# ljanyst/ssd-tensorflow

Hardware: AMD Instinct MI355X
Metric: images/sec (fwd+bwd) vgg300 batch32 (higher is better)
Workload: dtype f32; 1 GPU; vgg300 training step (forward + multibox loss + backward + momentum update), 32 images/GPU x 1 GPU, synthetic 300x300 BGR 0..255, GPU-encoded labels, Xavier-init weights (BASELINE.json configs[1]); global_batch=32, parallelism=dp1, allreduce=none

## Files before the change

### ssd_tensorflow_amd/csrc/api.hip

```cpp
#include "../../include/ssdvgg_hip.h"
#include "net.h"
#include "augment.h"
#include "annotate.h"
#include "jpeg.h"
#include "metrics.h"
#include <vector>
#include <map>
#include <memory>
#include <mutex>
#include <algorithm>

namespace ssd {
static thread_local std::string g_err;
void set_error(const char* fmt, ...) {
    char buf[1024];
    va_list ap;
    va_start(ap, fmt);
    vsnprintf(buf, sizeof buf, fmt, ap);
    va_end(ap);
    g_err = buf;
}
const char* get_error() { return g_err.c_str(); }

thread_local Profiler* g_prof = nullptr;
// ... 936 lines not shown
}
namespace {
struct WinoWs {
    float *U, *Uf, *V, *Mx, *Yt, *Ya, *slabs;
    size_t total;
    WinoWs(const ConvDesc& d, float* ws) {
        const size_t cop = wino_kpad(d.Co), u = (size_t)36 * d.Ci * cop, t = (size_t)36 * wino_tiles(d);
        U = ws; Uf = U + u; V = Uf + u; Mx = V + t * d.Ci; Yt = Mx + t * std::max((size_t)d.Ci, cop); Ya = Yt + t * cop; slabs = Ya + t * cop;
        total = (size_t)(slabs - ws) + wino_wgrad_ws_floats(d);
    }
};
}
size_t ssd_op_conv2d_wino_ws_floats(int b, int hi, int wi, int ci, int ho, int wo, int co, int kh, int kw, int stride, int dil,
                                    int pad_h, int pad_w) {
    const ConvDesc d = mk(b, hi, wi, ci, ho, wo, co, kh, kw, stride, dil, pad_h, pad_w);
    return wino_applicable(d) ? WinoWs(d, nullptr).total : 0;
}
size_t ssd_op_conv2d_wino_bits_words(int b, int hi, int wi, int ci, int ho, int wo, int co, int kh, int kw, int stride, int dil,
                                     int pad_h, int pad_w) {
    const ConvDesc d = mk(b, hi, wi, ci, ho, wo, co, kh, kw, stride, dil, pad_h, pad_w);
    return wino_applicable(d) ? (size_t)wino_tiles(d) * (d.Ci / 4) : 0;
}
int ssd_op_conv2d_wino_fwd(const float* x, const float* w, const float* bias, float* y, float* y_pool, void* rec, void* relu_bits, float* ws,
                           int flags, int b, int hi, int wi, int ci, int ho, int wo, int co, int kh, int kw, int stride, int dil,
                           int pad_h, int pad_w, int relu, void* stream) {
    API_BEGIN
    const ConvDesc d = mk(b, hi, wi, ci, ho, wo, co, kh, kw, stride, dil, pad_h, pad_w);
    SSD_REQUIRE(wino_applicable(d), "winograd: 3x3 / stride 1 / SAME layers (any dilation), Ci in multiples of 32, Co of 4");
    const WinoWs k(d, ws);
    if (!(flags & 1)) {
        HIP_OK(hipMemsetAsync(k.Uf, 0, (size_t)36 * d.Ci * wino_kpad(d.Co) * sizeof(float), (hipStream_t)stream));
        wino_filter(d, w, k.U, k.Uf, (hipStream_t)stream);
    }
    wino_fwd(d, x, k.U, bias, y, relu != 0, k.V, (size_t)wino_tiles(d) * d.Ci, k.Mx, y_pool, rec, (hipStream_t)stream, relu_bits);
    API_END
}
int ssd_op_conv2d_wino_dgrad(const float* dy, const float* w, float* dx, const float* mask, const void* mask_bits, int accumulate,
                             const void* rec, int uh, int uw, float* ws, int flags, int b, int hi, int wi, int ci, int ho, int wo, int co,
                             int kh, int kw, int stride, int dil, int pad_h, int pad_w, void* stream) {
    API_BEGIN
    const ConvDesc d = mk(b, hi, wi, ci, ho, wo, co, kh, kw, stride, dil, pad_h, pad_w);
    SSD_REQUIRE(wino_applicable(d), "winograd: 3x3 / stride 1 / SAME layers (any dilation), Ci in multiples of 32, Co of 4");
    const WinoWs k(d, ws);
    if (!(flags & 1)) {
        HIP_OK(hipMemsetAsync(k.Uf, 0, (size_t)36 * d.Ci * wino_kpad(d.Co) * sizeof(float), (hipStream_t)stream));
        wino_filter(d, w, k.U, k.Uf, (hipStream_t)stream);
    }
    wino_bwd_transform(d, dy, k.Yt, nullptr, (hipStream_t)stream);
    wino_dgrad(d, k.Yt, k.Uf, dx, mask, accumulate != 0, k.Mx, rec, uh, uw, (hipStream_t)stream, mask_bits);
    API_END
}
int ssd_op_conv2d_wino_wgrad(const float* x, const float* dy, float* dw, float* dbias, const float* w, float weight_decay, float* ws,
                             int flags, int b, int hi, int wi, int ci, int ho, int wo, int co, int kh, int kw, int stride, int dil,
                             int pad_h, int pad_w, void* stream) {
    API_BEGIN
    const ConvDesc d = mk(b, hi, wi, ci, ho, wo, co, kh, kw, stride, dil, pad_h, pad_w);
    SSD_REQUIRE(wino_applicable(d), "winograd: 3x3 / stride 1 / SAME layers (any dilation), Ci in multiples of 32, Co of 4");
    const WinoWs k(d, ws);
    const size_t vps = (size_t)wino_tiles(d) * d.Ci;
    if (!(flags & 2)) {
        ConvDesc dx = d;
        dx.Co = d.Ci; dx.Ho = d.Hi; dx.Wo = d.Wi;
        wino_bwd_transform(dx, x, k.V, nullptr, (hipStream_t)stream);
    }
    wino_bwd_transform(d, dy, nullptr, k.Ya, (hipStream_t)stream);
    wino_wgrad(d, k.V, vps, k.Ya, dw, dbias, w, weight_decay, k.slabs, (hipStream_t)stream);
    API_END
}
size_t ssd_op_conv2d_wgrad_ws_floats(int b, int hi, int wi, int ci, int ho, int wo, int co, int kh, int kw, int stride,
                                     int dil, int pad_h, int pad_w) {
    return conv_wgrad_ws_floats(mk(b, hi, wi, ci, ho, wo, co, kh, kw, stride, dil, pad_h, pad_w));
}
int ssd_op_conv2d_wgrad(const float* x, const float* dy, float* dw, float* dbias, const float* w, float weight_decay,
                        float* ws, int b, int hi, int wi, int ci, int ho, int wo, int co, int kh, int kw, int stride, int dil,
                        int pad_h, int pad_w, void* stream) {
    API_BEGIN
    conv_wgrad(mk(b, hi, wi, ci, ho, wo, co, kh, kw, stride, dil, pad_h, pad_w), x, dy, dw, dbias, w, weight_decay, ws,
               (hipStream_t)stream);
    API_END
}
int ssd_op_maxpool_fwd(const float* x, float* y, int b, int hi, int wi, int c, int ho, int wo, int k, int stride, int pad_h,
                       int pad_w, void* stream) {
// ... 167 lines not shown
```

### ssd_tensorflow_amd/csrc/conv.h

```cpp
#pragma once
#include <vector>
#include "common.h"

namespace ssd {

struct ConvDesc {
    int B, Hi, Wi, Ci;
    int Ho, Wo, Co;
    int KH, KW, stride, dil;
    int pad_h, pad_w;
};

void conv_fwd(const ConvDesc& d, const float* x, const float* w, const float* bias,
              float* y, bool relu, hipStream_t s);

void conv_dgrad(const ConvDesc& d, const float* dy, const float* w, float* dx,
                const float* mask, bool accumulate, hipStream_t s);

size_t conv_wgrad_ws_floats(const ConvDesc& d);
void conv_wgrad(const ConvDesc& d, const float* x, const float* dy, float* dw, float* dbias,
                const float* w, float weight_decay, float* ws, hipStream_t s);

bool conv_fwd_pool_supported(const ConvDesc& d);
void conv_fwd_pool(const ConvDesc& d, const float* x, const float* w, const float* bias, float* y_pool, void* rec, hipStream_t s);
bool conv_dgrad_unpool_supported(const ConvDesc& d);
void conv_dgrad_unpool(const ConvDesc& d, const float* dy, const float* w, float* dx_unpooled, const void* rec, int UH, int UW,
                       hipStream_t s);

bool conv_first_fwd_f32_applicable(const ConvDesc& d);
void conv_first_fwd_f32(const ConvDesc& d, const float* x, const float* w, const float* bias, float* y, bool relu, hipStream_t s);
bool conv_first_wgrad_f32_applicable(const ConvDesc& d);
size_t conv_first_wgrad_f32_ws_floats(const ConvDesc& d);
void conv_first_wgrad_f32(const ConvDesc& d, const float* x, const float* dy, float* dw, float* dbias, const float* w,
                          float weight_decay, float* ws, hipStream_t s);

bool wino_applicable(const ConvDesc& d);
int wino_tiles(const ConvDesc& d);
int wino_kpad(int c);
void wino_filter(const ConvDesc& d, const float* w, float* U, float* Uflip, hipStream_t s);
struct WinoFilterPlan {
    static constexpr int MAX = 24;
    struct Item {
        const float* w;
        float *U, *Uf;
        int Ci, Co, Cop, blk0;
    } it[MAX];
    int n = 0, blocks = 0;
    double elems = 0;
    void add(const float* w, float* U, float* Uf, int Ci, int Co);
};
void wino_filter_plan(const WinoFilterPlan& plan, bool forward, bool flipped, hipStream_t s);
size_t wino_fwd_ws_floats(const ConvDesc& d);
void wino_fwd(const ConvDesc& d, const float* x, const float* U, const float* bias, float* y, bool relu, float* V, size_t v_ps,
              float* Mws, float* y_pool, void* pool_rec, hipStream_t s, void* relu_bits = nullptr);
void wino_bwd_transform(const ConvDesc& d, const float* dy, float* Yt, float* Ya, hipStream_t s);
size_t wino_dgrad_ws_floats(const ConvDesc& d);
void wino_dgrad(const ConvDesc& d, const float* Yt, const float* Uflip, float* dx, const float* mask, bool accumulate, float* Xws,
                const void* unpool_rec, int UH, int UW, hipStream_t s, const void* mask_bits = nullptr);
size_t wino_wgrad_ws_floats(const ConvDesc& d);
void wino_wgrad(const ConvDesc& d, const float* V, size_t v_ps, const float* Ya, float* dw, float* dbias, const float* w,
                float weight_decay, float* ws, hipStream_t s);

bool conv_bigk(const ConvDesc& d);
double conv_bigk_useful_flops(const ConvDesc& d);
void conv_bigk_fwd(const ConvDesc& d, const float* x, const float* w, const float* bias, float* y, bool relu, hipStream_t s);
void conv_bigk_dgrad(const ConvDesc& d, const float* dy, const float* w, float* dx, const float* mask, bool accumulate, hipStream_t s);
void conv_bigk_wgrad(const ConvDesc& d, const float* x, const float* dy, float* dw, float* dbias, const float* w, float weight_decay,
                     hipStream_t s);

struct bf16_t;

void conv_fwd_smallc_bf16out(const ConvDesc& d, const float* x, const float* w, const float* bias, bf16_t* y, bool relu,
                             hipStream_t s);
void conv_wgrad_smallc_bf16dy(const ConvDesc& d, const float* x, const bf16_t* dy, float* dw, float* dbias, const float* w,
                              float weight_decay, float* ws, hipStream_t s);

void conv_first_fwd_bf16(const ConvDesc& d, const float* x, const float* w, const float* bias, bf16_t* y, bool relu, hipStream_t s);
size_t conv_first_wgrad_bf16_ws_floats(const ConvDesc& d);
void conv_first_wgrad_bf16(const ConvDesc& d, const float* x, const bf16_t* dy, float* dw, float* dbias, const float* w,
                           float weight_decay, float* ws, hipStream_t s);

void conv_bigk_fwd_bf16(const ConvDesc& d, const bf16_t* x, const bf16_t* w_oi, const float* bias, void* y, bool y_f32, bool relu,
                        hipStream_t s);
void conv_bigk_dgrad_bf16(const ConvDesc& d, const bf16_t* dy, const bf16_t* w_io, bf16_t* dx, const bf16_t* mask, bool accumulate,
                          hipStream_t s);
void conv_bigk_wgrad_bf16(const ConvDesc& d, const bf16_t* x, const bf16_t* dy, float* dw, float* dbias, const float* w,
                          float weight_decay, hipStream_t s);

struct FilterCastPlan {
    static constexpr int MAX_LAYERS = 48;
    struct Layer {
// ... 65 lines not shown
```

### ssd_tensorflow_amd/csrc/winograd.hip

```cpp
#include "conv.h"
#include "conv_detail.h"
#include "bf16.h"
#include <algorithm>
#include <cmath>

namespace ssd {

#define LDS_PTR(p) ((__attribute__((address_space(3))) void*)(p))
constexpr unsigned WOOB = 0xFFFFFFF0u;

__device__ __forceinline__ void bt6(f32x4& d0, f32x4& d1, f32x4& d2, f32x4& d3, f32x4& d4, f32x4& d5) {
    const f32x4 t0 = 1.265625f * d0 - 2.8125f * d2 + d4;
    const f32x4 e = d4 - 2.25f * d2, f = 1.6875f * d1 - 0.75f * d3;
    const f32x4 g = d4 - 0.5625f * d2, h = 0.84375f * d1 - 1.5f * d3;
    const f32x4 t5 = 1.265625f * d1 - 2.8125f * d3 + d5;
    d0 = t0; d1 = e - f; d2 = e + f; d3 = g - h; d4 = g + h; d5 = t5;
}
__device__ __forceinline__ void a6(const f32x4 e0, const f32x4 e1, const f32x4 e2, const f32x4 e3, f32x4* u) {
    const f32x4 p = e0 + 0.5625f * e2, q = 0.75f * e1 + 0.421875f * e3;
    const f32x4 r = e0 + 2.25f * e2, t = 1.5f * e1 + 3.375f * e3;
    u[0] = e0;
    u[1] = p + q;
    u[2] = p - q;
    u[3] = r + t;
    u[4] = r - t;
    u[5] = e3;
}
__device__ __forceinline__ void at4(const f32x4 m0, const f32x4 m1, const f32x4 m2, const f32x4 m3, const f32x4 m4, const f32x4 m5,
                                    f32x4* y) {
    const f32x4 s12 = m1 + m2, d12 = m1 - m2, s34 = m3 + m4, d34 = m3 - m4;
    y[0] = m0 + s12 + s34;
    y[1] = 0.75f * d12 + 1.5f * d34;
    y[2] = 0.5625f * s12 + 2.25f * s34;
    y[3] = 0.421875f * d12 + 3.375f * d34 + m5;
}

__host__ __device__ inline int bias_axis_slot(int k) { return k == 0 ? 0 : k == 1 ? 1 : k == 2 ? 2 : k == 5 ? 3 : -1; }
__device__ __forceinline__ float bias_axis_weight(int slot) {
    return slot == 0 ? -7.f / 9.f : slot == 1 ? 14.f / 9.f : slot == 2 ? 2.f / 9.f : 7.f / 16.f;
}

template <bool BT, bool AT>
__global__ __launch_bounds__(256) void wino_in_kernel(const float* __restrict__ x, float* __restrict__ V, float* __restrict__ Va,
                                                      int H, int W, int C, int Cp, int th, int tw, int T, unsigned x_bytes,
                                                      size_t v_ps, size_t va_ps, int D, unsigned long long* __restrict__ bits) {
    const int c4n = Cp >> 2;
    const int idx = blockIdx.x * 256 + threadIdx.x;
    const int q = idx % c4n, t = idx / c4n;
    if (t >= T) return;
    const int j = t % tw, t2 = t / tw;
    const int i = t2 % th, b = t2 / th;
    const int hb = (i % D) + D * 4 * (i / D), wb = (j % D) + D * 4 * (j / D);
    const __amdgpu_buffer_rsrc_t rs = __builtin_amdgcn_make_buffer_rsrc(const_cast<float*>(x), 0, x_bytes, 0x00020000);
    constexpr int LO = BT ? 0 : 1, HI = BT ? 6 : 5;
    f32x4 d[6][6];
#pragma unroll
    for (int r = LO; r < HI; ++r) {
        const int h = hb + D * (r - 1);
        const bool hv = (unsigned)h < (unsigned)H;
#pragma unroll
        for (int s = LO; s < HI; ++s) {
            const int w = wb + D * (s - 1);
            const bool ok = hv && (unsigned)w < (unsigned)W && q * 4 < C;
// ... 29 lines not shown
            a6(c[k][0], c[k][1], c[k][2], c[k][3], u);
#pragma unroll
            for (int l = 0; l < 6; ++l) *reinterpret_cast<f32x4*>(Va + (size_t)(k * 6 + l) * va_ps + row) = u[l];
        }
    }
    if constexpr (BT) {
#pragma unroll
        for (int s = 0; s < 6; ++s) bt6(d[0][s], d[1][s], d[2][s], d[3][s], d[4][s], d[5][s]);
#pragma unroll
        for (int r = 0; r < 6; ++r) {
            bt6(d[r][0], d[r][1], d[r][2], d[r][3], d[r][4], d[r][5]);
#pragma unroll
            for (int s = 0; s < 6; ++s) *reinterpret_cast<f32x4*>(V + (size_t)(r * 6 + s) * v_ps + row) = d[r][s];
        }
    }
}

struct WinoOutArgs {
    const float* M;
    size_t m_ps;
    float* y;
    const float* bias;
    const float* mask;
    const unsigned long long* mask_bits;
    int relu, accum;
    int H, W, N, th, tw, T;
    int D;
    unsigned short* pool_rec;
    int PH, PW;
    const unsigned short* unpool_rec;
    int UH, UW;
};

template <int MODE>
__global__ __launch_bounds__(256) void wino_out_kernel(WinoOutArgs p) {
    const int c4n = p.N >> 2;
    const int idx = blockIdx.x * 256 + threadIdx.x;
    const int q = idx % c4n, t = idx / c4n;
    if (t >= p.T) return;
    const int j = t % p.tw, t2 = t / p.tw;
    const int i = t2 % p.th, b = t2 / p.th;
    const int D = (MODE == 0 || MODE == 1) ? p.D : 1;
    const int hb = (i % D) + D * 4 * (i / D), wb = (j % D) + D * 4 * (j / D);
    const float* src = p.M + (size_t)t * p.N + q * 4;
    f32x4 c[4][6];
#pragma unroll
    for (int s = 0; s < 6; ++s) {
        f32x4 m[6];
#pragma unroll
        for (int r = 0; r < 6; ++r) m[r] = *reinterpret_cast<const f32x4*>(src + (size_t)(r * 6 + s) * p.m_ps);
        f32x4 y[4];
        at4(m[0], m[1], m[2], m[3], m[4], m[5], y);
#pragma unroll
        for (int r = 0; r < 4; ++r) c[r][s] = y[r];
    }
    f32x4 o[4][4];
#pragma unroll
    for (int r = 0; r < 4; ++r) at4(c[r][0], c[r][1], c[r][2], c[r][3], c[r][4], c[r][5], o[r]);

    if constexpr (MODE == 0 || MODE == 2) {
        const f32x4 bv = p.bias ? *reinterpret_cast<const f32x4*>(p.bias + q * 4) : f32x4{0.f, 0.f, 0.f, 0.f};
#pragma unroll
        for (int r = 0; r < 4; ++r)
#pragma unroll
            for (int s = 0; s < 4; ++s) {
                f32x4 v = o[r][s] + bv;
                if (p.relu) {
#pragma unroll
                    for (int e = 0; e < 4; ++e) v[e] = v[e] > 0.f ? v[e] : 0.f;
                }
                o[r][s] = v;
            }
    }
    if constexpr (MODE == 0) {
#pragma unroll
        for (int r = 0; r < 4; ++r) {
            const int h = hb + D * r;
            if (h >= p.H) continue;
#pragma unroll
            for (int s = 0; s < 4; ++s) {
                const int w = wb + D * s;
                if (w < p.W) *reinterpret_cast<f32x4*>(p.y + ((size_t)(b * p.H + h) * p.W + w) * p.N + q * 4) = o[r][s];
            }
        }
    } else if constexpr (MODE == 1) {
        const unsigned long long mbits = p.mask_bits ? p.mask_bits[(size_t)t * c4n + q] : 0ull;
#pragma unroll
        for (int r = 0; r < 4; ++r) {
            const int h = hb + D * r;
            if (h >= p.H) continue;
#pragma unroll
            for (int s = 0; s < 4; ++s) {
                const int w = wb + D * s;
                if (w >= p.W) continue;
                const size_t e0 = ((size_t)(b * p.H + h) * p.W + w) * p.N + q * 4;
                f32x4 v = o[r][s];
                if (p.accum) v += *reinterpret_cast<const f32x4*>(p.y + e0);
                if (p.mask_bits) {
                    const unsigned mb = (unsigned)(mbits >> ((r * 4 + s) * 4)) & 15u;
#pragma unroll
                    for (int e = 0; e < 4; ++e) v[e] = (mb >> e) & 1u ? v[e] : 0.f;
                } else if (p.mask) {
                    const f32x4 mk = *reinterpret_cast<const f32x4*>(p.mask + e0);
#pragma unroll
                    for (int e = 0; e < 4; ++e) v[e] = mk[e] > 0.f ? v[e] : 0.f;
                }
                *reinterpret_cast<f32x4*>(p.y + e0) = v;
            }
        }
    } else if constexpr (MODE == 2) {
#pragma unroll
        for (int wr = 0; wr < 2; ++wr) {
            const int ph = 2 * i + wr;
            if (ph >= p.PH) continue;
            const bool okh = 4 * i + 2 * wr + 1 < p.H;
#pragma unroll
            for (int wc = 0; wc < 2; ++wc) {
                const int pw = 2 * j + wc;
                if (pw >= p.PW) continue;
                const bool okw = 4 * j + 2 * wc + 1 < p.W;
                const bool ok[4] = {true, okw, okh, okw && okh};
                f32x4 mm = o[2 * wr][2 * wc];
                unsigned rec = 0;
#pragma unroll
                for (int e = 0; e < 4; ++e) {
                    unsigned a = 0;
                    float best = mm[e];
#pragma unroll
                    for (int cq = 1; cq < 4; ++cq) {
                        const float v = o[2 * wr + (cq >> 1)][2 * wc + (cq & 1)][e];
                        if (ok[cq] && v > best) { best = v; a = cq; }
                    }
                    mm[e] = best;
                    rec |= (a | (best > 0.f ? 4u : 0u)) << (3 * e);
                }
                const size_t pix = (size_t)(b * p.PH + ph) * p.PW + pw;
                *reinterpret_cast<f32x4*>(p.y + pix * p.N + q * 4) = mm;
                if (p.pool_rec) p.pool_rec[pix * c4n + q] = (unsigned short)rec;
            }
        }
    } else {
#pragma unroll
        for (int r = 0; r < 4; ++r) {
            const int h = 4 * i + r;
            if (h >= p.H) continue;
#pragma unroll
            for (int s = 0; s < 4; ++s) {
                const int w = 4 * j + s;
                if (w >= p.W) continue;
                const unsigned rec = p.unpool_rec[((size_t)(b * p.H + h) * p.W + w) * c4n + q];
#pragma unroll
                for (int cq = 0; cq < 4; ++cq) {
                    const int uh = 2 * h + (cq >> 1), uw = 2 * w + (cq & 1);
                    if (uh >= p.UH || uw >= p.UW) continue;
                    f32x4 v;
#pragma unroll
                    for (int e = 0; e < 4; ++e) {
                        const unsigned re = (rec >> (3 * e)) & 7u;
                        v[e] = ((re & 3u) == (unsigned)cq && (re & 4u)) ? o[r][s][e] : 0.f;
                    }
                    *reinterpret_cast<f32x4*>(p.y + ((size_t)(b * p.UH + uh) * p.UW + uw) * p.N + q * 4) = v;
                }
            }
        }
    }
}

__device__ __forceinline__ void g6(const float g0, const float g1, const float g2, float* u) {
    u[0] = (64.f / 81.f) * g0;
    const float a = (-128.f / 243.f) * g0 - (8.f / 27.f) * g2, b = (32.f / 81.f) * g1;
    u[1] = a - b;
    u[2] = a + b;
    const float c = (32.f / 243.f) * g0 + (8.f / 27.f) * g2, d = (16.f / 81.f) * g1;
    u[3] = c + d;
    u[4] = c - d;
    u[5] = g2;
}
template <bool FLIP>
__global__ __launch_bounds__(256) void wino_filter_kernel(WinoFilterPlan plan) {
    int li = 0;
    for (int k = 1; k < plan.n; ++k)
        if ((int)blockIdx.x >= plan.it[k].blk0) li = k;
    const float* __restrict__ w = plan.it[li].w;
    float* __restrict__ U = FLIP ? plan.it[li].Uf : plan.it[li].U;
    if (!U) return;
    const int Ci = plan.it[li].Ci, Co = plan.it[li].Co;
    const int idx = ((int)blockIdx.x - plan.it[li].blk0) * 256 + threadIdx.x;
    if (idx >= Ci * Co) return;
    const int ci = FLIP ? idx % Ci : idx / Co, co = FLIP ? idx / Ci : idx % Co;
    float g[3][3];
#pragma unroll
    for (int a = 0; a < 3; ++a)
#pragma unroll
        for (int b = 0; b < 3; ++b) g[a][b] = w[((size_t)((FLIP ? 2 - a : a) * 3 + (FLIP ? 2 - b : b)) * Ci + ci) * Co + co];
    float c[6][3];
#pragma unroll
    for (int b = 0; b < 3; ++b) {
        float u[6];
// ... 90 lines not shown
            for (int ni = 0; ni < TN; ++ni)
#pragma unroll
                for (int t = 0; t < 4; ++t) b[ni][t] = *reinterpret_cast<const float*>(S + b_col + ((kb + t) * BN + ni * 32) * 4);
#pragma unroll
            for (int t = 0; t < 4; ++t)
#pragma unroll
                for (int mi = 0; mi < TM; ++mi)
#pragma unroll
                    for (int ni = 0; ni < TN; ++ni)
                        acc[mi][ni] = __builtin_amdgcn_mfma_f32_32x32x2f32(a[mi][t], b[ni][t], acc[mi][ni], 0, 0, 0);
        }
    };
    if (nk > 0) issue(0, 0);
    for (int k = 0; k < nk; ++k) {
        asm volatile("s_waitcnt vmcnt(0)" ::: "memory");
        __builtin_amdgcn_s_barrier();
        asm volatile("" ::: "memory");
        if (k + 1 < nk) issue(k + 1, (k + 1) & 1);
        compute(k & 1);
    }
    float* const Cp = p.C + (size_t)pos * p.c_ps;
#pragma unroll
    for (int mi = 0; mi < TM; ++mi)
#pragma unroll
        for (int ni = 0; ni < TN; ++ni) {
            const int n = n0 + wn * 32 * TN + ni * 32 + li;
            if (n >= p.N) continue;
#pragma unroll
            for (int r = 0; r < 16; ++r) {
                const int m = m0 + wm * 32 * TM + mi * 32 + (r & 3) + 8 * (r >> 2) + 4 * lh;
                if (m < p.M) Cp[(size_t)m * p.N + n] = acc[mi][ni][r];
            }
        }
}

struct WinoTnArgs {
    const float* X;
    const float* Y;
    float* ws;
    int T, Ci, Co;
    int x_ld, y_ld;
    size_t x_ps, y_ps;
    int CT, NT, tchunk, nsplit;
};

template <int WM, int WN, int TM, int TN>
__global__ __launch_bounds__(256) void wino_gemm_tn_kernel(WinoTnArgs p) {
    constexpr int BKT = 32 * TM * WM, BNT = 32 * TN * WN, BP = 32;
    constexpr int XC = BKT / 4, YC = BNT / 4;
    constexpr int XRPP = 256 / XC, YRPP = 256 / YC;
    constexpr int X_N = BP / XRPP, Y_N = BP / YRPP;
    constexpr int X_BYTES = BP * BKT * 4, STAGE = BP * (BKT + BNT) * 4;
    static_assert(WM * WN == 4, "4 waves per workgroup");
    extern __shared__ __attribute__((aligned(16))) float smem[];
    unsigned char* const lds = reinterpret_cast<unsigned char*>(smem);
    const int tid = threadIdx.x;
    const int wave = __builtin_amdgcn_readfirstlane(tid >> 6), lane = tid & 63;
    int wg = xcd_remap(blockIdx.x, gridDim.x);
    const int nt = wg % p.NT;
    wg /= p.NT;
    const int ct = wg % p.CT;
    wg /= p.CT;
    const int split = wg % p.nsplit, pos = wg / p.nsplit;
    const int c0 = ct * BKT, n0 = nt * BNT;
    const int tbeg = split * p.tchunk, tend = min(p.T, tbeg + p.tchunk);
    const int niter = (tend - tbeg + BP - 1) / BP;
// ... 220 lines not shown
    static bool once = (set_lds(kern, lds), true);
    (void)once;
    a.MT = cdiv(a.M, BM);
    a.NT = cdiv(a.N, BN);
    ProfScope prof(label, 2.0 * 36 * a.M * (double)a.N * a.K, 4.0 * 36 * ((double)a.M * a.K + (double)a.K * a.N + (double)a.M * a.N), s);
    hipLaunchKernelGGL(kern, dim3(36 * a.MT * a.NT), dim3(256), lds, s, a);
    HIP_OK(hipGetLastError());
}

static void gemm_nn(const float* A, size_t a_ps, const float* Bm, float* C, size_t c_ps, int M, int N, int K, hipStream_t s) {
    WinoGemmArgs a{};
    a.A = A; a.Bm = Bm; a.C = C; a.M = M; a.N = N; a.K = K;
    a.a_ps = a_ps; a.b_ps = (size_t)K * N; a.c_ps = c_ps;
    static const int forced = env_int("SSD_WINO_TILE", -1);
    int cfg = 0;
    if (forced >= 0) cfg = forced;
    else if (cdiv(N, 64) * 64 < cdiv(N, 128) * 128) cfg = 1;
    else if ((double)cdiv(M, 128) * 128 > 1.06 * M && (double)cdiv(M, 64) * 64 < (double)cdiv(M, 128) * 128) cfg = 2;
    switch (cfg) {
    case 0: launch_nn<2, 2, 2, 2>(a, "wino_gemm_128x128", s); break;
    case 1: launch_nn<4, 1, 1, 2>(a, "wino_gemm_128x64", s); break;
    case 2: launch_nn<2, 2, 1, 2>(a, "wino_gemm_64x128", s); break;
    default: launch_nn<2, 2, 1, 1>(a, "wino_gemm_64x64", s); break;
    }
}

template <int MODE>
static void launch_out(WinoOutArgs& a, const char* label, double bytes, hipStream_t s) {
    ProfScope prof(label, 0, bytes, s);
    SSD_LAUNCH_STOP(wino_out_kernel<MODE>, dim3(cdiv((long long)a.T * (a.N / 4), 256)), dim3(256), 0, s, a);
    HIP_OK(hipGetLastError());
}

size_t wino_fwd_ws_floats(const ConvDesc& d) { return (size_t)36 * wino_tiles(d) * d.Co; }

void wino_fwd(const ConvDesc& d, const float* x, const float* U, const float* bias, float* y, bool relu, float* V, size_t v_ps,
              float* Mws, float* y_pool, void* pool_rec, hipStream_t s, void* relu_bits) {
    require(d);
    const int T = wino_tiles(d);
    launch_in(x, V, nullptr, d.B, d.Hi, d.Wi, d.Ci, d.Ci, d.dil, v_ps, 0, s, static_cast<unsigned long long*>(relu_bits));
    gemm_nn(V, v_ps, U, Mws, (size_t)T * d.Co, T, d.Co, d.Ci, s);
    WinoOutArgs a{};
    a.M = Mws; a.m_ps = (size_t)T * d.Co; a.bias = bias; a.relu = relu; a.H = d.Ho; a.W = d.Wo; a.N = d.Co;
    a.th = tiles_1d(d.Ho, d.dil); a.tw = tiles_1d(d.Wo, d.dil); a.T = T; a.D = d.dil;
    const double mb = 4.0 * 36 * T * d.Co;
    if (y_pool) {
        SSD_REQUIRE(d.dil == 1, "winograd: the fused pool is for undilated layers");
        a.y = y_pool; a.pool_rec = static_cast<unsigned short*>(pool_rec); a.PH = (d.Ho + 1) / 2; a.PW = (d.Wo + 1) / 2;
        launch_out<2>(a, "wino_out_pool", mb + 4.0 * d.B * a.PH * a.PW * d.Co, s);
    } else {
        a.y = y;
        launch_out<0>(a, "wino_out", mb + 4.0 * d.B * d.Ho * d.Wo * d.Co, s);
    }
}

size_t wino_dgrad_ws_floats(const ConvDesc& d) { return (size_t)36 * wino_tiles(d) * d.Ci; }

void wino_bwd_transform(const ConvDesc& d, const float* dy, float* Yt, float* Ya, hipStream_t s) {
    require(d);
    const size_t ps = (size_t)wino_tiles(d) * wino_kpad(d.Co);
    launch_in(dy, Yt, Ya, d.B, d.Ho, d.Wo, d.Co, wino_kpad(d.Co), d.dil, ps, ps, s);
}

void wino_dgrad(const ConvDesc& d, const float* Yt, const float* Uflip, float* dx, const float* mask, bool accumulate, float* Xws,
                const void* unpool_rec, int UH, int UW, hipStream_t s, const void* mask_bits) {
    require(d);
    const int T = wino_tiles(d);
    gemm_nn(Yt, (size_t)T * wino_kpad(d.Co), Uflip, Xws, (size_t)T * d.Ci, T, d.Ci, wino_kpad(d.Co), s);
    WinoOutArgs a{};
    a.M = Xws; a.m_ps = (size_t)T * d.Ci; a.y = dx; a.mask = mask; a.accum = accumulate; a.H = d.Hi; a.W = d.Wi; a.N = d.Ci;
    a.mask_bits = mask ? static_cast<const unsigned long long*>(mask_bits) : nullptr;
    a.th = tiles_1d(d.Hi, d.dil); a.tw = tiles_1d(d.Wi, d.dil); a.T = T; a.D = d.dil;
    const double mb = 4.0 * 36 * T * d.Ci;
    if (unpool_rec) {
        SSD_REQUIRE(d.dil == 1, "winograd: the un-pooling form is for undilated layers");
        a.unpool_rec = static_cast<const unsigned short*>(unpool_rec); a.UH = UH; a.UW = UW;
        launch_out<3>(a, "wino_out_unpool", mb + 4.0 * d.B * UH * UW * d.Ci, s);
    } else {
        launch_out<1>(a, "wino_out_dgrad", mb + 4.0 * d.B * d.Hi * d.Wi * d.Ci * (mask && !a.mask_bits ? 2 : 1), s);
    }
}

static void tn_tile(const ConvDesc& d, int* bk, int* bn) {
    *bk = d.Ci <= 64 ? 64 : 128;
    *bn = d.Co <= 64 ? 64 : 128;
}
static int tn_splits(const ConvDesc& d) {
    const int T = wino_tiles(d);
    int bk, bn;
    tn_tile(d, &bk, &bn);
    const int base = 36 * cdiv(d.Ci, bk) * cdiv(d.Co, bn);
    const double slots = 256.0 * std::min(8, (int)(160 * 1024 / (2 * 32 * (bk + bn) * 4)));
    const double it_us = 3.4 * (bk * bn) / (128.0 * 128.0) * slots / 512.0;
    int best = 1;
    double bc = 1e300;
    for (int ns = 1; ns <= 16; ++ns) {
        const int chunk = cdiv(cdiv(T, ns), 32) * 32;
        if (ns > 1 && chunk < 128) break;
        const double rounds = std::ceil((double)base * ns / slots);
        const double cost = rounds * (chunk / 32) * it_us + (ns > 1 ? 2.0 * ns * 36.0 * d.Ci * d.Co * 4.0 / 4.0e6 : 0.0);
        if (cost < bc) { bc = cost; best = ns; }
    }
    return best;
}
size_t wino_wgrad_ws_floats(const ConvDesc& d) { return (size_t)tn_splits(d) * ((size_t)36 * d.Ci * d.Co + 16 * (size_t)d.Co); }

template <int WM, int WN, int TM, int TN>
static void launch_tn(WinoTnArgs& a, const char* label, double flops, double bytes, hipStream_t s) {
    constexpr int BKT = 32 * TM * WM, BNT = 32 * TN * WN;
    constexpr size_t lds = 2 * (size_t)32 * (BKT + BNT) * 4;
    auto kern = wino_gemm_tn_kernel<WM, WN, TM, TN>;
    static bool once = (set_lds(kern, lds), true);
// ... 36 lines not shown
```

Before: 1364 images/s.

## Fuse Winograd batched GEMM with output transform for small-channel layers

Adds a new MFMA kernel that runs all 36 Winograd-domain GEMMs for a 32x64 output tile, keeps the 36 accumulators in registers, and then applies the inverse transform, bias/ReLU, pooling, masking or unpooling in the same kernel. It replaces the separate gemm_nn plus wino_out launch for undilated layers whose channel sizes are 64/128 (excluding 128x128), in both forward and dgrad. This removes the round trip of the 36xTxN intermediate through global memory and one launch. The cost is heavy register pressure (36 f32x4 accumulators) with 512-thread blocks, which may limit occupancy. The path can be disabled through an environment variable or a flag bit.

```diff
diff --git a/ssd_tensorflow_amd/csrc/api.hip b/ssd_tensorflow_amd/csrc/api.hip
--- a/ssd_tensorflow_amd/csrc/api.hip
+++ b/ssd_tensorflow_amd/csrc/api.hip
@@ -992,7 +992,8 @@
         HIP_OK(hipMemsetAsync(k.Uf, 0, (size_t)36 * d.Ci * wino_kpad(d.Co) * sizeof(float), (hipStream_t)stream));
         wino_filter(d, w, k.U, k.Uf, (hipStream_t)stream);
     }
-    wino_fwd(d, x, k.U, bias, y, relu != 0, k.V, (size_t)wino_tiles(d) * d.Ci, k.Mx, y_pool, rec, (hipStream_t)stream, relu_bits);
+    wino_fwd(d, x, k.U, bias, y, relu != 0, k.V, (size_t)wino_tiles(d) * d.Ci, k.Mx, y_pool, rec, (hipStream_t)stream, relu_bits,
+             (flags & 4) != 0);
     API_END
 }
 int ssd_op_conv2d_wino_dgrad(const float* dy, const float* w, float* dx, const float* mask, const void* mask_bits, int accumulate,
@@ -1007,7 +1008,7 @@
         wino_filter(d, w, k.U, k.Uf, (hipStream_t)stream);
     }
     wino_bwd_transform(d, dy, k.Yt, nullptr, (hipStream_t)stream);
-    wino_dgrad(d, k.Yt, k.Uf, dx, mask, accumulate != 0, k.Mx, rec, uh, uw, (hipStream_t)stream, mask_bits);
+    wino_dgrad(d, k.Yt, k.Uf, dx, mask, accumulate != 0, k.Mx, rec, uh, uw, (hipStream_t)stream, mask_bits, (flags & 4) != 0);
     API_END
 }
 int ssd_op_conv2d_wino_wgrad(const float* x, const float* dy, float* dw, float* dbias, const float* w, float weight_decay, float* ws,
diff --git a/ssd_tensorflow_amd/csrc/conv.h b/ssd_tensorflow_amd/csrc/conv.h
--- a/ssd_tensorflow_amd/csrc/conv.h
+++ b/ssd_tensorflow_amd/csrc/conv.h
@@ -52,11 +52,11 @@
 void wino_filter_plan(const WinoFilterPlan& plan, bool forward, bool flipped, hipStream_t s);
 size_t wino_fwd_ws_floats(const ConvDesc& d);
 void wino_fwd(const ConvDesc& d, const float* x, const float* U, const float* bias, float* y, bool relu, float* V, size_t v_ps,
-              float* Mws, float* y_pool, void* pool_rec, hipStream_t s, void* relu_bits = nullptr);
+              float* Mws, float* y_pool, void* pool_rec, hipStream_t s, void* relu_bits = nullptr, bool two_launch = false);
 void wino_bwd_transform(const ConvDesc& d, const float* dy, float* Yt, float* Ya, hipStream_t s);
 size_t wino_dgrad_ws_floats(const ConvDesc& d);
 void wino_dgrad(const ConvDesc& d, const float* Yt, const float* Uflip, float* dx, const float* mask, bool accumulate, float* Xws,
-                const void* unpool_rec, int UH, int UW, hipStream_t s, const void* mask_bits = nullptr);
+                const void* unpool_rec, int UH, int UW, hipStream_t s, const void* mask_bits = nullptr, bool two_launch = false);
 size_t wino_wgrad_ws_floats(const ConvDesc& d);
 void wino_wgrad(const ConvDesc& d, const float* V, size_t v_ps, const float* Ya, float* dw, float* dbias, const float* w,
                 float weight_decay, float* ws, hipStream_t s);
diff --git a/ssd_tensorflow_amd/csrc/winograd.hip b/ssd_tensorflow_amd/csrc/winograd.hip
--- a/ssd_tensorflow_amd/csrc/winograd.hip
+++ b/ssd_tensorflow_amd/csrc/winograd.hip
@@ -26,9 +26,9 @@
     u[4] = r - t;
     u[5] = e3;
 }
-__device__ __forceinline__ void at4(const f32x4 m0, const f32x4 m1, const f32x4 m2, const f32x4 m3, const f32x4 m4, const f32x4 m5,
-                                    f32x4* y) {
-    const f32x4 s12 = m1 + m2, d12 = m1 - m2, s34 = m3 + m4, d34 = m3 - m4;
+template <class V>
+__device__ __forceinline__ void at4(const V m0, const V m1, const V m2, const V m3, const V m4, const V m5, V* y) {
+    const V s12 = m1 + m2, d12 = m1 - m2, s34 = m3 + m4, d34 = m3 - m4;
     y[0] = m0 + s12 + s34;
     y[1] = 0.75f * d12 + 1.5f * d34;
     y[2] = 0.5625f * s12 + 2.25f * s34;
@@ -124,46 +124,46 @@
     int UH, UW;
 };
 
+template <class F>
+__device__ __forceinline__ void wino_out_transform(F m, f32x4 (&o)[4][4]) {
+    typedef f32x4 V;
+    V c[4][6];
+#pragma unroll
+    for (int s = 0; s < 6; ++s) {
+        V mm[6];
+#pragma unroll
+        for (int r = 0; r < 6; ++r) mm[r] = m(r, s);
+        V y[4];
+        at4(mm[0], mm[1], mm[2], mm[3], mm[4], mm[5], y);
+#pragma unroll
+        for (int r = 0; r < 4; ++r) c[r][s] = y[r];
+    }
+#pragma unroll
+    for (int r = 0; r < 4; ++r) at4(c[r][0], c[r][1], c[r][2], c[r][3], c[r][4], c[r][5], o[r]);
+}
+
+__device__ __forceinline__ void wino_out_bias_relu(f32x4 (&o)[4][4], const f32x4 bv, int relu) {
+#pragma unroll
+    for (int r = 0; r < 4; ++r)
+#pragma unroll
+        for (int s = 0; s < 4; ++s) {
+            f32x4 v = o[r][s] + bv;
+            if (relu) {
+#pragma unroll
+                for (int e = 0; e < 4; ++e) v[e] = v[e] > 0.f ? v[e] : 0.f;
+            }
+            o[r][s] = v;
+        }
+}
+
 template <int MODE>
-__global__ __launch_bounds__(256) void wino_out_kernel(WinoOutArgs p) {
-    const int c4n = p.N >> 2;
-    const int idx = blockIdx.x * 256 + threadIdx.x;
-    const int q = idx % c4n, t = idx / c4n;
-    if (t >= p.T) return;
+__device__ __forceinline__ void wino_out_store(const WinoOutArgs& p, int t, int q, f32x4 (&o)[4][4]) {
+    typedef f32x4 V;
+    const int c4n = p.N >> 2, ch = q * 4;
     const int j = t % p.tw, t2 = t / p.tw;
     const int i = t2 % p.th, b = t2 / p.th;
     const int D = (MODE == 0 || MODE == 1) ? p.D : 1;
     const int hb = (i % D) + D * 4 * (i / D), wb = (j % D) + D * 4 * (j / D);
-    const float* src = p.M + (size_t)t * p.N + q * 4;
-    f32x4 c[4][6];
-#pragma unroll
-    for (int s = 0; s < 6; ++s) {
-        f32x4 m[6];
-#pragma unroll
-        for (int r = 0; r < 6; ++r) m[r] = *reinterpret_cast<const f32x4*>(src + (size_t)(r * 6 + s) * p.m_ps);
-        f32x4 y[4];
-        at4(m[0], m[1], m[2], m[3], m[4], m[5], y);
-#pragma unroll
-        for (int r = 0; r < 4; ++r) c[r][s] = y[r];
-    }
-    f32x4 o[4][4];
-#pragma unroll
-    for (int r = 0; r < 4; ++r) at4(c[r][0], c[r][1], c[r][2], c[r][3], c[r][4], c[r][5], o[r]);
-
-    if constexpr (MODE == 0 || MODE == 2) {
-        const f32x4 bv = p.bias ? *reinterpret_cast<const f32x4*>(p.bias + q * 4) : f32x4{0.f, 0.f, 0.f, 0.f};
-#pragma unroll
-        for (int r = 0; r < 4; ++r)
-#pragma unroll
-            for (int s = 0; s < 4; ++s) {
-                f32x4 v = o[r][s] + bv;
-                if (p.relu) {
-#pragma unroll
-                    for (int e = 0; e < 4; ++e) v[e] = v[e] > 0.f ? v[e] : 0.f;
-                }
-                o[r][s] = v;
-            }
-    }
     if constexpr (MODE == 0) {
 #pragma unroll
         for (int r = 0; r < 4; ++r) {
@@ -172,7 +172,7 @@
 #pragma unroll
             for (int s = 0; s < 4; ++s) {
                 const int w = wb + D * s;
-                if (w < p.W) *reinterpret_cast<f32x4*>(p.y + ((size_t)(b * p.H + h) * p.W + w) * p.N + q * 4) = o[r][s];
+                if (w < p.W) *reinterpret_cast<V*>(p.y + ((size_t)(b * p.H + h) * p.W + w) * p.N + ch) = o[r][s];
             }
         }
     } else if constexpr (MODE == 1) {
@@ -185,19 +185,19 @@
             for (int s = 0; s < 4; ++s) {
                 const int w = wb + D * s;
                 if (w >= p.W) continue;
-                const size_t e0 = ((size_t)(b * p.H + h) * p.W + w) * p.N + q * 4;
-                f32x4 v = o[r][s];
-                if (p.accum) v += *reinterpret_cast<const f32x4*>(p.y + e0);
+                const size_t e0 = ((size_t)(b * p.H + h) * p.W + w) * p.N + ch;
+                V v = o[r][s];
+                if (p.accum) v += *reinterpret_cast<const V*>(p.y + e0);
                 if (p.mask_bits) {
                     const unsigned mb = (unsigned)(mbits >> ((r * 4 + s) * 4)) & 15u;
 #pragma unroll
                     for (int e = 0; e < 4; ++e) v[e] = (mb >> e) & 1u ? v[e] : 0.f;
                 } else if (p.mask) {
-                    const f32x4 mk = *reinterpret_cast<const f32x4*>(p.mask + e0);
+                    const V mk = *reinterpret_cast<const V*>(p.mask + e0);
 #pragma unroll
                     for (int e = 0; e < 4; ++e) v[e] = mk[e] > 0.f ? v[e] : 0.f;
                 }
-                *reinterpret_cast<f32x4*>(p.y + e0) = v;
+                *reinterpret_cast<V*>(p.y + e0) = v;
             }
         }
     } else if constexpr (MODE == 2) {
@@ -212,7 +212,7 @@
                 if (pw >= p.PW) continue;
                 const bool okw = 4 * j + 2 * wc + 1 < p.W;
                 const bool ok[4] = {true, okw, okh, okw && okh};
-                f32x4 mm = o[2 * wr][2 * wc];
+                V mm = o[2 * wr][2 * wc];
                 unsigned rec = 0;
 #pragma unroll
                 for (int e = 0; e < 4; ++e) {
@@ -227,7 +227,7 @@
                     rec |= (a | (best > 0.f ? 4u : 0u)) << (3 * e);
                 }
                 const size_t pix = (size_t)(b * p.PH + ph) * p.PW + pw;
-                *reinterpret_cast<f32x4*>(p.y + pix * p.N + q * 4) = mm;
+                *reinterpret_cast<V*>(p.y + pix * p.N + ch) = mm;
                 if (p.pool_rec) p.pool_rec[pix * c4n + q] = (unsigned short)rec;
             }
         }
@@ -245,17 +245,31 @@
                 for (int cq = 0; cq < 4; ++cq) {
                     const int uh = 2 * h + (cq >> 1), uw = 2 * w + (cq & 1);
                     if (uh >= p.UH || uw >= p.UW) continue;
-                    f32x4 v;
+                    V v;
 #pragma unroll
                     for (int e = 0; e < 4; ++e) {
                         const unsigned re = (rec >> (3 * e)) & 7u;
                         v[e] = ((re & 3u) == (unsigned)cq && (re & 4u)) ? o[r][s][e] : 0.f;
                     }
-                    *reinterpret_cast<f32x4*>(p.y + ((size_t)(b * p.UH + uh) * p.UW + uw) * p.N + q * 4) = v;
+                    *reinterpret_cast<V*>(p.y + ((size_t)(b * p.UH + uh) * p.UW + uw) * p.N + ch) = v;
                 }
             }
         }
     }
+}
+
+template <int MODE>
+__global__ __launch_bounds__(256) void wino_out_kernel(WinoOutArgs p) {
+    const int c4n = p.N >> 2;
+    const int idx = blockIdx.x * 256 + threadIdx.x;
+    const int q = idx % c4n, t = idx / c4n;
+    if (t >= p.T) return;
+    const float* src = p.M + (size_t)t * p.N + q * 4;
+    f32x4 o[4][4];
+    wino_out_transform([&](int r, int s) { return *reinterpret_cast<const f32x4*>(src + (size_t)(r * 6 + s) * p.m_ps); }, o);
+    if constexpr (MODE == 0 || MODE == 2)
+        wino_out_bias_relu(o, p.bias ? *reinterpret_cast<const f32x4*>(p.bias + q * 4) : f32x4{0.f, 0.f, 0.f, 0.f}, p.relu);
+    wino_out_store<MODE>(p, t, q, o);
 }
 
 __device__ __forceinline__ void g6(const float g0, const float g1, const float g2, float* u) {
@@ -412,6 +426,117 @@
                 if (m < p.M) Cp[(size_t)m * p.N + n] = acc[mi][ni][r];
             }
         }
+}
+
+struct WinoFusedArgs {
+    const float* A;
+    const float* Bm;
+    int M, N, K;
+    size_t a_ps, b_ps;
+    int NT;
+    WinoOutArgs out;
+};
+
+template <int MODE, int KS>
+__global__ __launch_bounds__(512) void wino_gemm_out_kernel(WinoFusedArgs p) {
+    constexpr int NS = 4, total = 36 * KS, A_BYTES = 32 * 64 * 4, B_BYTES = 64 * 64 * 4, STAGE = A_BYTES + B_BYTES;
+    extern __shared__ __attribute__((aligned(16))) float smem[];
+    unsigned char* const lds = reinterpret_cast<unsigned char*>(smem);
+    const int tid = threadIdx.x;
+    const int wave = __builtin_amdgcn_readfirstlane(tid >> 6), lane = tid & 63;
+    const int wg = xcd_remap(blockIdx.x, gridDim.x);
+    const int nt = wg % p.NT, mt = wg / p.NT;
+    const int m0 = mt * 32, n0 = nt * 64;
+
+    const int ar = (tid & 255) >> 3;
+    const unsigned a_off = m0 + ar < p.M ? (unsigned)((m0 + ar) * p.K + (tid >> 8) * 32 + (((tid & 7) ^ ((ar >> 1) & 7)) * 4)) * 4u : WOOB;
+    unsigned b_off[2];
+#pragma unroll
+    for (int j = 0; j < 2; ++j) {
+        const int k = (j * 8 + wave) * 4 + (lane >> 4);
+        b_off[j] = (unsigned)(k * p.N + n0 + (((lane & 15) ^ ((wave & 1) * 4)) * 4)) * 4u;
+    }
+    const unsigned a_bytes = (unsigned)((size_t)p.M * p.K * 4u), b_bytes = (unsigned)((size_t)p.K * p.N * 4u);
+    auto issue = [&](int st) {
+        const int pos = st / KS, kh = st % KS;
+        const __amdgpu_buffer_rsrc_t a_rs = __builtin_amdgcn_make_buffer_rsrc(const_cast<float*>(p.A + (size_t)pos * p.a_ps), 0, a_bytes, 0x00020000);
+        const __amdgpu_buffer_rsrc_t b_rs = __builtin_amdgcn_make_buffer_rsrc(const_cast<float*>(p.Bm + (size_t)pos * p.b_ps), 0, b_bytes, 0x00020000);
+        unsigned char* S = lds + (st & (NS - 1)) * STAGE + wave * 1024;
+        __builtin_amdgcn_raw_ptr_buffer_load_lds(a_rs, LDS_PTR(S), 16, (int)a_off, kh * 256, 0, 0);
+#pragma unroll
+        for (int j = 0; j < 2; ++j)
+            __builtin_amdgcn_raw_ptr_buffer_load_lds(b_rs, LDS_PTR(S + A_BYTES + j * 8192), 16, (int)b_off[j], kh * 64 * p.N * 4, 0, 0);
+    };
+
+    const int tb = wave >> 2, cb = wave & 3;
+    const int li = lane & 15, ks = lane >> 4;
+    const bool khi = ks >> 1;
+    const int row = tb * 16 + li;
+    const int a_row = row * 128 + (((ks & 1) ^ ((row >> 1) & 7)) * 16);
+    const int b_col = A_BYTES + ((ks & 1) * 4 + (ks >> 1)) * 256 + (((cb * 4 + (li >> 2)) ^ ((ks & 1) * 4)) * 16) + (li & 3) * 4;
+    struct Frag {
+        f32x4 v[4];
+        float u[4][2];
+    };
+    auto fetch = [&](int st, int half, Frag& f) {
+        const unsigned char* S = lds + (st & (NS - 1)) * STAGE;
+#pragma unroll
+        for (int g = 0; g < 4; ++g) {
+            f.v[g] = *reinterpret_cast<const f32x4*>(S + half * 4096 + (a_row ^ (g * 32)));
+            f.u[g][0] = *reinterpret_cast<const float*>(S + b_col + (half * 32 + g * 8) * 256);
+            f.u[g][1] = *reinterpret_cast<const float*>(S + b_col + (half * 32 + g * 8 + 2) * 256);
+        }
+    };
+    auto mma = [&](const Frag& f, f32x4& acc) {
+#pragma unroll
+        for (int g = 0; g < 4; ++g) {
+            acc = __builtin_amdgcn_mfma_f32_16x16x4f32(f.u[g][0], khi ? f.v[g][1] : f.v[g][0], acc, 0, 0, 0);
+            acc = __builtin_amdgcn_mfma_f32_16x16x4f32(f.u[g][1], khi ? f.v[g][3] : f.v[g][2], acc, 0, 0, 0);
+        }
+    };
+    auto arrive = [&](int st) {
+        if (st + NS - 2 < total) asm volatile("s_waitcnt vmcnt(6) lgkmcnt(0)" ::: "memory");
+        else asm volatile("s_waitcnt vmcnt(0) lgkmcnt(0)" ::: "memory");
+        __builtin_amdgcn_s_barrier();
+        asm volatile("" ::: "memory");
+        if (st + NS - 1 < total) issue(st + NS - 1);
+    };
+
+    f32x4 acc[36];
+#pragma unroll
+    for (int i = 0; i < 36; ++i) acc[i] = f32x4{0.f, 0.f, 0.f, 0.f};
+#pragma unroll
+    for (int st = 0; st < NS - 1; ++st) issue(st);
+    Frag f0, f1;
+    arrive(0);
+    fetch(0, 0, f0);
+#pragma unroll
+    for (int pos = 0; pos < 36; ++pos) {
+#pragma unroll
+        for (int kh = 0; kh < KS; ++kh) {
+            const int it = pos * KS + kh;
+            fetch(it, 1, f1);
+            __builtin_amdgcn_sched_barrier(0);
+            mma(f0, acc[pos]);
+            __builtin_amdgcn_sched_barrier(0);
+            if (it + 1 < total) {
+                arrive(it + 1);
+                fetch(it + 1, 0, f0);
+            }
+            __builtin_amdgcn_sched_barrier(0);
+            mma(f1, acc[pos]);
+            __builtin_amdgcn_sched_barrier(0);
+        }
+    }
+
+    const int t = m0 + tb * 16 + li;
+    if (t >= p.out.T) return;
+    const int q = (n0 >> 2) + cb * 4 + ks;
+    f32x4 o[4][4];
+    wino_out_transform([&](int r, int s) { return acc[r * 6 + s]; }, o);
+    if constexpr (MODE == 0 || MODE == 2)
+        wino_out_bias_relu(o, p.out.bias ? *reinterpret_cast<const f32x4*>(p.out.bias + q * 4) : f32x4{0.f, 0.f, 0.f, 0.f}, p.out.relu);
+    wino_out_store<MODE>(p.out, t, q, o);
 }
 
 struct WinoTnArgs {
@@ -698,14 +823,39 @@
     HIP_OK(hipGetLastError());
 }
 
+static bool fuse_out(const ConvDesc& d, int N, int K, bool two_launch) {
+    static const int on = env_int("SSD_WINO_FUSE_OUT", 1);
+    return on && !two_launch && d.dil == 1 && (N == 64 || N == 128) && (K == 64 || K == 128) && !(N == 128 && K == 128);
+}
+template <int MODE>
+static void launch_fused(const float* A, size_t a_ps, const float* Bm, int K, const WinoOutArgs& o, double out_bytes, hipStream_t s) {
+    constexpr size_t lds = 4 * (size_t)(32 * 64 + 64 * 64) * 4;
+    WinoFusedArgs a{};
+    a.A = A; a.Bm = Bm; a.M = o.T; a.N = o.N; a.K = K; a.a_ps = a_ps; a.b_ps = (size_t)K * o.N; a.NT = o.N / 64; a.out = o;
+    ProfScope prof("wino_gemm_out_32x64", 2.0 * 36 * a.M * (double)a.N * a.K, 4.0 * 36 * ((double)a.M * a.K + (double)a.K * a.N) + out_bytes, s);
+    if (K == 64) {
+        auto kern = wino_gemm_out_kernel<MODE, 1>;
+        static bool once = (set_lds(kern, lds), true);
+        (void)once;
+        SSD_LAUNCH_STOP(kern, dim3(cdiv(a.M, 32) * a.NT), dim3(512), lds, s, a);
+    } else {
+        auto kern = wino_gemm_out_kernel<MODE, 2>;
+        static bool once = (set_lds(kern, lds), true);
+        (void)once;
+        SSD_LAUNCH_STOP(kern, dim3(cdiv(a.M, 32) * a.NT), dim3(512), lds, s, a);
+    }
+    HIP_OK(hipGetLastError());
+}
+
 size_t wino_fwd_ws_floats(const ConvDesc& d) { return (size_t)36 * wino_tiles(d) * d.Co; }
 
 void wino_fwd(const ConvDesc& d, const float* x, const float* U, const float* bias, float* y, bool relu, float* V, size_t v_ps,
-              float* Mws, float* y_pool, void* pool_rec, hipStream_t s, void* relu_bits) {
+              float* Mws, float* y_pool, void* pool_rec, hipStream_t s, void* relu_bits, bool two_launch) {
     require(d);
     const int T = wino_tiles(d);
     launch_in(x, V, nullptr, d.B, d.Hi, d.Wi, d.Ci, d.Ci, d.dil, v_ps, 0, s, static_cast<unsigned long long*>(relu_bits));
-    gemm_nn(V, v_ps, U, Mws, (size_t)T * d.Co, T, d.Co, d.Ci, s);
+    const bool fused = fuse_out(d, d.Co, d.Ci, two_launch);
+    if (!fused) gemm_nn(V, v_ps, U, Mws, (size_t)T * d.Co, T, d.Co, d.Ci, s);
     WinoOutArgs a{};
     a.M = Mws; a.m_ps = (size_t)T * d.Co; a.bias = bias; a.relu = relu; a.H = d.Ho; a.W = d.Wo; a.N = d.Co;
     a.th = tiles_1d(d.Ho, d.dil); a.tw = tiles_1d(d.Wo, d.dil); a.T = T; a.D = d.dil;
@@ -713,10 +863,14 @@
     if (y_pool) {
         SSD_REQUIRE(d.dil == 1, "winograd: the fused pool is for undilated layers");
         a.y = y_pool; a.pool_rec = static_cast<unsigned short*>(pool_rec); a.PH = (d.Ho + 1) / 2; a.PW = (d.Wo + 1) / 2;
-        launch_out<2>(a, "wino_out_pool", mb + 4.0 * d.B * a.PH * a.PW * d.Co, s);
+        const double ob = 4.0 * d.B * a.PH * a.PW * d.Co;
+        if (fused) launch_fused<2>(V, v_ps, U, d.Ci, a, ob, s);
+        else launch_out<2>(a, "wino_out_pool", mb + ob, s);
     } else {
         a.y = y;
-        launch_out<0>(a, "wino_out", mb + 4.0 * d.B * d.Ho * d.Wo * d.Co, s);
+        const double ob = 4.0 * d.B * d.Ho * d.Wo * d.Co;
+        if (fused) launch_fused<0>(V, v_ps, U, d.Ci, a, ob, s);
+        else launch_out<0>(a, "wino_out", mb + ob, s);
     }
 }
 
@@ -729,10 +883,12 @@
 }
 
 void wino_dgrad(const ConvDesc& d, const float* Yt, const float* Uflip, float* dx, const float* mask, bool accumulate, float* Xws,
-                const void* unpool_rec, int UH, int UW, hipStream_t s, const void* mask_bits) {
+                const void* unpool_rec, int UH, int UW, hipStream_t s, const void* mask_bits, bool two_launch) {
     require(d);
     const int T = wino_tiles(d);
-    gemm_nn(Yt, (size_t)T * wino_kpad(d.Co), Uflip, Xws, (size_t)T * d.Ci, T, d.Ci, wino_kpad(d.Co), s);
+    const size_t yt_ps = (size_t)T * wino_kpad(d.Co);
+    const bool fused = fuse_out(d, d.Ci, wino_kpad(d.Co), two_launch);
+    if (!fused) gemm_nn(Yt, yt_ps, Uflip, Xws, (size_t)T * d.Ci, T, d.Ci, wino_kpad(d.Co), s);
     WinoOutArgs a{};
     a.M = Xws; a.m_ps = (size_t)T * d.Ci; a.y = dx; a.mask = mask; a.accum = accumulate; a.H = d.Hi; a.W = d.Wi; a.N = d.Ci;
     a.mask_bits = mask ? static_cast<const unsigned long long*>(mask_bits) : nullptr;
@@ -741,9 +897,13 @@
     if (unpool_rec) {
         SSD_REQUIRE(d.dil == 1, "winograd: the un-pooling form is for undilated layers");
         a.unpool_rec = static_cast<const unsigned short*>(unpool_rec); a.UH = UH; a.UW = UW;
-        launch_out<3>(a, "wino_out_unpool", mb + 4.0 * d.B * UH * UW * d.Ci, s);
+        const double ob = 4.0 * d.B * UH * UW * d.Ci;
+        if (fused) launch_fused<3>(Yt, yt_ps, Uflip, wino_kpad(d.Co), a, ob, s);
+        else launch_out<3>(a, "wino_out_unpool", mb + ob, s);
     } else {
-        launch_out<1>(a, "wino_out_dgrad", mb + 4.0 * d.B * d.Hi * d.Wi * d.Ci * (mask && !a.mask_bits ? 2 : 1), s);
+        const double ob = 4.0 * d.B * d.Hi * d.Wi * d.Ci * (mask && !a.mask_bits ? 2 : 1);
+        if (fused) launch_fused<1>(Yt, yt_ps, Uflip, wino_kpad(d.Co), a, ob, s);
+        else launch_out<1>(a, "wino_out_dgrad", mb + ob, s);
     }
 }
 
```

Result: faster. 1413 images/s, median of 6 (+3.6%).
